# mikhaildubov/AST-text-analysis

Measured on AMD Instinct MI355X. Metric: corpus chars/sec (SA+annotation build + keyphrase score table), higher is better.
Workload: dtype u32 (symbols/indices) + f64 (scores); 1 GPU; 1 synthetic 64 MiB random-ASCII word-stream doc(s) per GPU (text mode), 1000 keyphrases, normalized scores, easa-HIP; symbols_per_gpu=61142967, strings_per_gpu=2982949, parallelism=doc-shard x1, all_gather_bytes_per_rank=0

## Files before the change

### ast-text-analysis_amd/csrc/build.h

```cpp
#pragma once
#include "dc3.h"
#include "score.h"
#include "tables.h"
#include "upload.h"
#include <chrono>

static bool kgram_reserve(east_hip_index *h, u64 bins, u32 n_docs);

static void annotate(east_hip_index *h, Ctx &ctx)
{
    const Pyramid &pyr = h->pyr;
    const u32 n = pyr.len[0];
    Arena &ar = *ctx.arena;
    const size_t mark = ar.mark();
    const u32 n_tiles = ceil_div_u32(n, ANN_TILE);
    u32 *wide_list = ar.alloc<u32>((size_t)n_tiles * ANN_TILE);
    u32 *wide_count = ar.alloc<u32>(n_tiles);
    const bool has_lvl1 = pyr.levels > 1;
    LAUNCH(ctx, ann_stream_kernel, n_tiles, pyr.ptr[0], (const u32 *)h->doc_off, (const u32 *)h->n_strings,
           h->build_docs, n, h->ann, has_lvl1 ? (u32 *)pyr.ptr[1] : (u32 *)nullptr, has_lvl1 ? pyr.len[1] : 0u,
           has_lvl1 ? pyr_padded(pyr.len[1]) : 0u, wide_list, wide_count, h->lcp);
    int l = 2;
    for (; l < pyr.levels && pyr.len[l] > PYR_TOP; l++)
        LAUNCH(ctx, pyramid_level_kernel, ceil_div_u32(pyr_padded(pyr.len[l]), BLOCK), pyr.ptr[l - 1], pyr.len[l],
               pyr_padded(pyr.len[l]), (u32 *)pyr.ptr[l]);
    if (l < pyr.levels) LAUNCH(ctx, pyramid_top_kernel, 1, pyr, l);
    LAUNCH(ctx, ann_wide_kernel, ceil_div_u32(n_tiles, BLOCK / ANN_WIDE_SLOTS), pyr, n, n_tiles, (const u32 *)wide_list,
           (const u32 *)wide_count, h->ann);
    ar.release(mark);
}

__global__ __launch_bounds__(BLOCK) void byte_hist_kernel(const uint8_t *__restrict__ s8, u32 n, u32 *__restrict__ counts)
{
    __shared__ u32 bins[4][256];
    for (int c = 0; c < 4; c++) bins[c][threadIdx.x] = 0;
    __syncthreads();
    u32 *mine = bins[threadIdx.x & 3u];
    for (u64 i = ((u64)blockIdx.x * BLOCK + threadIdx.x) * 16u; i < n; i += (u64)gridDim.x * BLOCK * 16u) {
        const uint4 x = *reinterpret_cast<const uint4 *>(s8 + i);
        const u32 wds[4] = {x.x, x.y, x.z, x.w};
#pragma unroll
        for (int q = 0; q < 16; q++)
            if (i + q < n) atomicAdd(&mine[(wds[q >> 2] >> ((q & 3) * 8)) & 0xFFu], 1u);
    }
    __syncthreads();
    const u32 t = bins[0][threadIdx.x] + bins[1][threadIdx.x] + bins[2][threadIdx.x] + bins[3][threadIdx.x];
    if (t) atomicAdd(&counts[threadIdx.x], t);
}

static void prepare_ht_code(east_hip_index *h, Ctx &ctx, u32 n, u32 sigma_t, u32 m_total)
{
    ctx.ht_max_len = 0;
    if (ctx.dry || !h->use_s8 || !ctx.knobs.window_sort || ctx.knobs.ht_mode == 0) return;
    if (ctx.spec) {
        if (!h->ht_valid || h->ht_sigma != sigma_t) {
            if (ctx.knobs.ht_mode == 1 && sigma_t + 1 >= 8 && n >= 64) throw SpecAbort();
            return;
        }
    } else {
        h->ht_valid = false;
        if (sigma_t + 1 < 8 || (ctx.knobs.ht_mode != 1 && (bit_width_u32(sigma_t + 1) < 6 || n < 65536)) || n < 64) return;
// ... 528 lines not shown
```

### ast-text-analysis_amd/csrc/debug_api.h

```cpp
#pragma once

struct DebugScope {
    hipStream_t stream = nullptr;
    Arena arena;
    Stats stats;
    Ctx ctx;
    DebugScope(int device, size_t bytes)
    {
        int c = 0;
        if (hipGetDeviceCount(&c) != hipSuccess || c <= 0)
            east_throw(EAST_HIP_ERR_NO_DEVICE, "no HIP device available (this library has no CPU fallback)");
        if (device < 0 || device >= c) east_throw(EAST_HIP_ERR_NO_DEVICE, "device ordinal out of range");
        use_device_ordinal(device);
        HIP_CHECK(hipStreamCreateWithFlags(&stream, hipStreamNonBlocking));
        void *p = nullptr;
        HIP_CHECK(hipMalloc(&p, bytes));
        arena.base = (char *)p;
        arena.cap = bytes;
        ctx.stream = stream;
        ctx.arena = &arena;
        ctx.stats = &stats;
    }
    ~DebugScope()
    {
// ... 35 lines not shown
    Arena &ar = sc.arena;
    u32 *d_sym = ar.alloc<u32>(n), *d_map = ar.alloc<u32>(TEXT_SYMBOLS);
    HIP_CHECK(hipMemcpyAsync(d_sym, symbols, (size_t)n * 4, hipMemcpyHostToDevice, sc.stream));
    HIP_CHECK(hipMemcpyAsync(d_map, code_map, TEXT_SYMBOLS * 4, hipMemcpyHostToDevice, sc.stream));
    for (int v = 0; v < 2; v++) {
        uint8_t *s8 = ar.alloc<uint8_t>((size_t)n + 64);
        u32 *present = ar.alloc<u32>(PRESENT_WORDS + 1), *hist = ar.alloc<u32>(hist_words), *group_sum = ar.alloc<u32>(sum_words);
        u32 *total = ar.alloc<u32>(total_words);
        HIP_CHECK(hipMemsetAsync(s8, v ? 0xA5 : 0x5A, (size_t)n + 64, sc.stream));
        HIP_CHECK(hipMemsetAsync(present, 0, (PRESENT_WORDS + 1) * 4, sc.stream));
        HIP_CHECK(hipMemsetAsync(hist, 0xEE, hist_words * 4, sc.stream));
        HIP_CHECK(hipMemsetAsync(group_sum, 0xEE, sum_words * 4, sc.stream));
        HIP_CHECK(hipMemsetAsync(total, 0, total_words * 4, sc.stream));
        const TextWindowGen<K> gen{s8, n, w, b, spare, term_first, DocKey()};
        if (v == 0) {
            LAUNCH_NAMED(sc.ctx, "presence_remap_hist_kernel", (presence_remap_hist_kernel<K, TextWindowGen<K>>), n_groups,
                         (const u32 *)d_sym, n, (const u32 *)d_map, present, s8, gen, shift, mask, n_tiles, hist, group_sum, total);
        } else {
            LAUNCH(sc.ctx, presence_kernel, std::min<u32>(ceil_div_u32(n, BLOCK), 2048), (const u32 *)d_sym, n, 1, present);
            LAUNCH(sc.ctx, remap_bytes_kernel, ceil_div_u32((u64)n + 16, BLOCK * 16), (const u32 *)d_sym, (const u32 *)d_map, n, 1, s8);
            hipLaunchKernelGGL((radix_hist_kernel<K, TextWindowGen<K>, false>), dim3(n_groups), dim3(RS_HIST_THREADS), 0, sc.stream, gen, n,
                               shift, mask, n_tiles, hist, group_sum, total, RsSeg());
            HIP_CHECK(hipGetLastError());
        }
        HIP_CHECK(hipMemcpyAsync(s8_out + (size_t)v * ((size_t)n + 16), s8, (size_t)n + 16, hipMemcpyDeviceToHost, sc.stream));
        HIP_CHECK(hipMemcpyAsync(present_out + (size_t)v * PRESENT_WORDS, present, PRESENT_WORDS * 4, hipMemcpyDeviceToHost, sc.stream));
        HIP_CHECK(hipMemcpyAsync(hist_out + v * hist_words, hist, hist_words * 4, hipMemcpyDeviceToHost, sc.stream));
        HIP_CHECK(hipMemcpyAsync(group_sum_out + v * sum_words, group_sum, sum_words * 4, hipMemcpyDeviceToHost, sc.stream));
        HIP_CHECK(hipMemcpyAsync(digit_total_out + v * total_words, total, total_words * 4, hipMemcpyDeviceToHost, sc.stream));
    }
    HIP_CHECK(hipStreamSynchronize(sc.stream));
}

extern "C" {

int east_hip_debug_set_rank_bucket_bytes(int64_t bytes)
{
    if (bytes < 0) return EAST_HIP_ERR_INVALID;
    knobs_update([&](Knobs &k) { k.rank_bucket_bytes = (size_t)bytes; k.plan_epoch++; });
    return EAST_HIP_OK;
}

int east_hip_debug_set_window_sort(int enabled)
{
    knobs_update([&](Knobs &k) {
    k.window_sort = enabled != 0;
    k.force_lean = enabled == 2;
    k.force_wide_keys = enabled == 3 || enabled == 5;
    k.fused_finish = enabled != 4 && enabled != 5 && enabled != 9 && getenv("EAST_HIP_NO_FUSED_FINISH") == nullptr;
    k.force_fused = enabled == 6 || getenv("EAST_HIP_FORCE_FUSED") != nullptr;
    k.ht_mode = enabled == 7 || enabled == 9 ? 1 : enabled == 8 ? 0 : env_int("EAST_HIP_HT", -1);
    k.plan_epoch++;
    });
    return EAST_HIP_OK;
}

int east_hip_debug_set_segmented_sort(int mode)
{
    knobs_update([&](Knobs &k) { k.seg_mode = mode < 0 ? env_int("EAST_HIP_SEG", -1) : (mode != 0); k.plan_epoch++; });
    return EAST_HIP_OK;
}

int east_hip_debug_alphabetic_code(const uint64_t *weights, int32_t n, uint32_t *code, int32_t *len)
{
    if (!weights || !code || !len || n < 1) return EAST_HIP_ERR_INVALID;
    std::vector<u64> w(weights, weights + n);
// ... 65 lines not shown

int east_hip_debug_set_text_stream(int64_t chunk_bytes)
{
    knobs_update([&](Knobs &k) { k.tp_stream = chunk_bytes; });
    return EAST_HIP_OK;
}

int east_hip_debug_set_score_path(int mode)
{
    knobs_update([&](Knobs &k) {
        k.kg_pairs = mode == 1 || mode == 2 || mode == 4 || mode == 5;
        k.kg_pairs_forced = mode == 4;
        k.score_fused = mode == 1 || mode == 3 || mode == 4 || mode == 5;
        k.score_endgame = mode == 5 ? 0 : 1;
    });
    return EAST_HIP_OK;
}

int east_hip_debug_set_speculation(int enabled)
{
    knobs_update([&](Knobs &k) { k.speculate = enabled != 0; k.first_hist = enabled != 2 && getenv("EAST_HIP_NO_FIRST_HIST") == nullptr; });
    return EAST_HIP_OK;
}

int east_hip_debug_first_pass_hist(int device, const uint32_t *symbols, int64_t n, const uint32_t *code_map, int key_bytes,
                                   int w, int b, int spare, uint32_t term_first, int shift, uint32_t mask, uint8_t *s8,
                                   uint32_t *present, uint32_t *hist, uint32_t *group_sum, uint32_t *digit_total)
{
    return guarded([&] {
        if (key_bytes == 8) debug_first_pass_hist<u64>(device, symbols, n, code_map, w, b, spare, term_first, shift, mask, s8, present, hist, group_sum, digit_total);
        else if (key_bytes == 4) debug_first_pass_hist<u32>(device, symbols, n, code_map, w, b, spare, term_first, shift, mask, s8, present, hist, group_sum, digit_total);
        else east_throw(EAST_HIP_ERR_INVALID, "key_bytes must be 4 or 8");
    });
}

int east_hip_debug_radix_sort_u64(int device, uint64_t *keys, uint32_t *vals, int64_t n, int bits)
{
    return guarded([&] { debug_sort<u64>(device, keys, vals, n, bits); });
}

int east_hip_debug_radix_sort_u32(int device, uint32_t *keys, uint32_t *vals, int64_t n, int bits)
{
    return guarded([&] { debug_sort<u32>(device, keys, vals, n, bits); });
}

int east_hip_debug_exclusive_scan(int device, const uint32_t *in, uint32_t *out, int64_t n)
{
    return guarded([&] {
        if (n < 0 || n >= (i64)0x7FFFFFF0 || !in || !out) east_throw(EAST_HIP_ERR_INVALID, "bad scan arguments");
        if (n == 0) return;
        DebugScope sc(device, (size_t)n * 8 + (size_t)ceil_div_u32(n, SCAN_TILE) * 16 + (8u << 20));
        u32 *d_in = sc.arena.alloc<u32>(n), *d_out = sc.arena.alloc<u32>(n);
        HIP_CHECK(hipMemcpyAsync(d_in, in, (size_t)n * 4, hipMemcpyHostToDevice, sc.stream));
        device_scan<ArrIn, false>(sc.ctx, ArrIn{d_in}, (u32)n, d_out);
        HIP_CHECK(hipMemcpyAsync(out, d_out, (size_t)n * 4, hipMemcpyDeviceToHost, sc.stream));
        HIP_CHECK(hipStreamSynchronize(sc.stream));
    });
}

int east_hip_debug_suffix_array(int device, const uint32_t *symbols, int64_t n, uint32_t sigma, int32_t *sa_out,
                                int32_t *levels_out)
{
    return guarded([&] {
        if (n < 1 || n >= (i64)0x7FFFFFF0 || !symbols || !sa_out || sigma < 1)
            east_throw(EAST_HIP_ERR_INVALID, "bad suffix array arguments");
        for (i64 i = 0; i < n; i++)
// ... 24 lines not shown
```

### ast-text-analysis_amd/csrc/tables.h

```cpp
#pragma once
#include "common.h"

#define PYR_SHIFT 4
#define PYR_FAN 16u
#define PYR_MAX_LEVELS 9
#define NONE_U32 0xFFFFFFFFu

struct Pyramid {
    const u32 *ptr[PYR_MAX_LEVELS];
    u32 len[PYR_MAX_LEVELS];
    int levels;
};

static inline u32 pyr_padded(u32 len) { return (len + PYR_FAN - 1u) & ~(PYR_FAN - 1u); }
__device__ __forceinline__ u32 pyr_padded_dev(u32 len) { return (len + PYR_FAN - 1u) & ~(PYR_FAN - 1u); }

__device__ __forceinline__ u32 doc_of(const u32 *__restrict__ doc_off, u32 n_docs, u32 x)
{
    u32 lo = 0, hi = n_docs;
    while (hi - lo > 1) {
        const u32 mid = (lo + hi) >> 1;
        if (doc_off[mid] <= x) lo = mid; else hi = mid;
    }
    return lo;
// ... 429 lines not shown
            rlvl--;
        }
    }
    pse = lq;
    nsv = rq;
}

__device__ __forceinline__ u32 pyr_leftmost_argmin(const Pyramid &P, u32 a, u32 b)
{
    const u32 lo = a + 1;
    u32 best = NONE_U32;
    {
        u32 l = lo, h = b;
        int lvl = 0;
        while (l < h) {
            const u32 *M = P.ptr[lvl];
            while (l < h && (l & (PYR_FAN - 1u))) { const u32 x = M[l]; best = x < best ? x : best; l++; }
            while (l < h && (h & (PYR_FAN - 1u))) { h--; const u32 x = M[h]; best = x < best ? x : best; }
            if (l >= h) break;
            if (lvl + 1 >= P.levels) {
                for (u32 q = l; q < h; q++) { const u32 x = M[q]; best = x < best ? x : best; }
                break;
            }
            l >>= PYR_SHIFT; h >>= PYR_SHIFT; lvl++;
        }
    }
    if (P.ptr[0][lo] == best) return lo;
    return pyr_find_right<false>(P, lo, best);
}

#ifndef ANN_NEAR
#define ANN_NEAR 8
#endif
#define ANN_IPT 4
#define ANN_TILE (BLOCK * ANN_IPT)
#ifndef ANN_HALO
#define ANN_HALO 64
#endif
#ifndef ANN_LOCAL
#define ANN_LOCAL 64
#endif

__global__ __launch_bounds__(BLOCK) void ann_stream_kernel(const u32 *__restrict__ lcp, const u32 *__restrict__ doc_off,
                                                           const u32 *__restrict__ n_strings, u32 n_docs, u32 n,
                                                           u32 *__restrict__ ann, u32 *__restrict__ lvl1, u32 len1,
                                                           u32 len1_padded, u32 *__restrict__ wide_list,
                                                           u32 *__restrict__ wide_count,
                                                           u32 *__restrict__ lcp_pad)
{
    __shared__ __attribute__((aligned(16))) u32 tile[ANN_TILE + 2 * ANN_HALO];
    __shared__ u32 work[ANN_TILE];
    __shared__ u32 work_count, far_count;
    if (threadIdx.x == 0) { work_count = 0; far_count = 0; }
    if (lcp_pad && blockIdx.x == gridDim.x - 1 && threadIdx.x < PYR_FAN && n + threadIdx.x < ((n + PYR_FAN - 1u) & ~(PYR_FAN - 1u)))
        lcp_pad[n + threadIdx.x] = NONE_U32;
    const u32 tile_base = blockIdx.x * ANN_TILE;
    const u32 k0 = tile_base + threadIdx.x * ANN_IPT;
    {
        uint4 x = {0u, 0u, 0u, 0u};
        if (k0 < ((n + PYR_FAN - 1u) & ~(PYR_FAN - 1u))) x = *reinterpret_cast<const uint4 *>(lcp + k0);
        if (k0 + 0 >= n) x.x = 0u;
        if (k0 + 1 >= n) x.y = 0u;
        if (k0 + 2 >= n) x.z = 0u;
        if (k0 + 3 >= n) x.w = 0u;
        const bool has_halo = threadIdx.x < 2 * ANN_HALO / 4;
        const bool left = threadIdx.x < ANN_HALO / 4;
        const u32 q = left ? threadIdx.x : threadIdx.x - ANN_HALO / 4;
        const i64 g = left ? (i64)tile_base - ANN_HALO + 4 * q : (i64)tile_base + ANN_TILE + 4 * q;
        uint4 h = {0u, 0u, 0u, 0u};
        if (has_halo && g >= 0 && g < (i64)((n + PYR_FAN - 1u) & ~(PYR_FAN - 1u))) h = *reinterpret_cast<const uint4 *>(lcp + g);
        *reinterpret_cast<uint4 *>(&tile[ANN_HALO + threadIdx.x * ANN_IPT]) = x;
        if (has_halo) {
            if (g + 0 >= (i64)n) h.x = 0u;
            if (g + 1 >= (i64)n) h.y = 0u;
            if (g + 2 >= (i64)n) h.z = 0u;
            if (g + 3 >= (i64)n) h.w = 0u;
            *reinterpret_cast<uint4 *>(&tile[left ? 4 * q : ANN_HALO + ANN_TILE + 4 * q]) = h;
        }
    }
    __syncthreads();
    if (threadIdx.x < ANN_TILE / PYR_FAN) {
        const u32 e = tile_base / PYR_FAN + threadIdx.x;
        if (e < len1_padded) {
            u32 m = NONE_U32;
            if (e < len1) {
                const uint4 *g = reinterpret_cast<const uint4 *>(&tile[ANN_HALO + threadIdx.x * PYR_FAN]);
#pragma unroll
                for (int q = 0; q < 4; q++) {
                    const uint4 y = g[q];
                    const u32 r = e * PYR_FAN + 4u * q;
                    if (r + 0 < n) m = min(m, y.x);
                    if (r + 1 < n) m = min(m, y.y);
                    if (r + 2 < n) m = min(m, y.z);
                    if (r + 3 < n) m = min(m, y.w);
                }
            }
            lvl1[e] = m;
        }
    }
    if (k0 < n) {
        u32 c[ANN_IPT + 2 * ANN_NEAR];
#pragma unroll
        for (int q = 0; q < (ANN_IPT + 2 * ANN_NEAR) / 4; q++) {
            const uint4 x = *reinterpret_cast<const uint4 *>(&tile[ANN_HALO + threadIdx.x * ANN_IPT - ANN_NEAR + 4 * q]);
            c[4 * q] = x.x; c[4 * q + 1] = x.y; c[4 * q + 2] = x.z; c[4 * q + 3] = x.w;
        }
        u32 out[ANN_IPT];
        bool direct[ANN_IPT];
#pragma unroll
        for (int e = 0; e < ANN_IPT; e++) {
            const u32 k = k0 + e;
            const int i = ANN_NEAR + e;
            const u32 v = c[i];
            out[e] = 0;
            direct[e] = true;
            if (k >= n) continue;
            if (v == 0) {
                const u32 d = n_docs > 1 ? doc_of(doc_off, n_docs, k) : 0u;
                out[e] = doc_off[d] == k ? (doc_off[d + 1] - k) - n_strings[d] : 0u;
                continue;
            }
            u32 back = 0, x = 0;
#pragma unroll
            for (int t = ANN_NEAR; t >= 1; t--)
                if (c[i - t] <= v) { back = (u32)t; x = c[i - t]; }
            if (back == 0) { direct[e] = false; continue; }
            if (x < v) {
                u32 fwd = 0;
#pragma unroll
                for (int t = ANN_NEAR; t >= 1; t--)
                    if (c[i + t] < v) fwd = (u32)t;
                if (fwd == 0) direct[e] = false;
                else out[e] = fwd + back;
            }
        }
        if (direct[0] && direct[1] && direct[2] && direct[3] && k0 + ANN_IPT <= n) {
            *reinterpret_cast<uint4 *>(ann + k0) = uint4{out[0], out[1], out[2], out[3]};
        } else {
#pragma unroll
            for (int e = 0; e < ANN_IPT; e++) {
                if (k0 + e >= n) break;
                if (direct[e]) ann[k0 + e] = out[e];
                else work[atomicAdd(&work_count, 1u)] = threadIdx.x * ANN_IPT + e;
            }
        }
    }
    __syncthreads();
    const u32 count = work_count;
    const u32 sub = threadIdx.x & 7u;
    for (u32 wi = threadIdx.x >> 3; wi < count; wi += BLOCK / 8) {
        const u32 local = work[wi], at = ANN_HALO + local;
        const u32 v = tile[at];
        constexpr u32 NONE_D = ANN_LOCAL + 1;
        u32 d = NONE_D;
#pragma unroll
        for (u32 t = 0; t < (ANN_LOCAL + 7) / 8; t++) {
            const u32 dist = 1u + sub + 8u * t;
            if (dist <= ANN_LOCAL && d == NONE_D && tile[at - dist] <= v) d = dist;
        }
        d = min(d, (u32)__shfl_xor((int)d, 1, 8));
        d = min(d, (u32)__shfl_xor((int)d, 2, 8));
        d = min(d, (u32)__shfl_xor((int)d, 4, 8));
        bool far = d == NONE_D;
        u32 a = 0;
        if (!far && tile[at - d] < v) {
            u32 e = NONE_D;
#pragma unroll
            for (u32 t = 0; t < (ANN_LOCAL + 7) / 8; t++) {
                const u32 dist = 1u + sub + 8u * t;
                if (dist <= ANN_LOCAL && e == NONE_D && tile[at + dist] < v) e = dist;
            }
            e = min(e, (u32)__shfl_xor((int)e, 1, 8));
            e = min(e, (u32)__shfl_xor((int)e, 2, 8));
            e = min(e, (u32)__shfl_xor((int)e, 4, 8));
            if (e == NONE_D) far = true;
            else a = d + e;
        }
        if (sub == 0) {
            if (far) wide_list[tile_base + atomicAdd(&far_count, 1u)] = tile_base + local;
            else ann[tile_base + local] = a;
        }
    }
    __syncthreads();
    if (threadIdx.x == 0) wide_count[blockIdx.x] = far_count;
}

#define ANN_WIDE_SLOTS 16
__global__ __launch_bounds__(BLOCK) void ann_wide_kernel(Pyramid P, u32 n, u32 n_tiles, const u32 *__restrict__ wide_list,
                                                         const u32 *__restrict__ wide_count, u32 *__restrict__ ann)
{
    const u32 *lcp = P.ptr[0];
    const u32 tile = blockIdx.x * (BLOCK / ANN_WIDE_SLOTS) + threadIdx.x / ANN_WIDE_SLOTS;
    if (tile >= n_tiles) return;
    const u32 count = wide_count[tile];
    for (u32 i = threadIdx.x % ANN_WIDE_SLOTS; i < count; i += ANN_WIDE_SLOTS) {
        const u32 k = wide_list[tile * ANN_TILE + i];
        const u32 v = lcp[k];
        u32 pse, nsv;
        pyr_find_both(P, k, v, pse, nsv);
        u32 a = 0;
        if (pse != NONE_U32 && lcp[pse] < v) a = (nsv == NONE_U32 ? n : nsv) - pse;
        ann[k] = a;
    }
}

#define CH_NEAR 8
#ifndef CH_HALO
#define CH_HALO 64
#endif
#ifndef CH_LOCAL
#define CH_LOCAL 64
#endif
#define CH_IPT 4
#define CH_TILE (BLOCK * CH_IPT)

__device__ __forceinline__ void child_of_rank(const Pyramid &P, u32 k, u32 seg, u32 seg_end, u32 &u, u32 &dn, u32 &nx)
{
    const u32 *lcp = P.ptr[0];
    const u32 v = lcp[k];
    u32 pse = NONE_U32, nse = NONE_U32;
    if (k > seg) {
        pse = pyr_find_left<false>(P, k, v);
        if (pse != NONE_U32 && pse < seg) pse = NONE_U32;
    }
    nse = pyr_find_right<false>(P, k, v);
    if (nse != NONE_U32 && nse >= seg_end) nse = NONE_U32;
    nx = (nse != NONE_U32 && lcp[nse] == v) ? nse - seg : 0u;
    u = dn = 0;
    if (pse != NONE_U32 && k - pse > 1) u = pyr_leftmost_argmin(P, pse, k) - seg;
    if (nse != NONE_U32 && nse - k > 1) dn = pyr_leftmost_argmin(P, k, nse) - seg;
}

__global__ __launch_bounds__(BLOCK) void child_stream_kernel(Pyramid P, const u32 *__restrict__ doc_off, u32 n_docs, u32 n,
                                                             u32 *__restrict__ up, u32 *__restrict__ down,
                                                             u32 *__restrict__ next, u32 *__restrict__ wide_list,
                                                             u32 *__restrict__ wide_count)
{
// ... 228 lines not shown
```

### ast-text-analysis_amd/east/hip_backend.py

```python
import atexit
import ctypes
import os

import numpy as np

from east import exceptions

_HERE = os.path.dirname(os.path.abspath(__file__))
LIB_PATH = os.environ.get("EAST_HIP_LIBRARY", os.path.join(_HERE, "_lib", "libeast_hip.so"))

_c_i64p = ctypes.POINTER(ctypes.c_int64)
_c_i32p = ctypes.POINTER(ctypes.c_int32)
_c_u32p = ctypes.POINTER(ctypes.c_uint32)
_c_u64p = ctypes.POINTER(ctypes.c_uint64)
_c_dblp = ctypes.POINTER(ctypes.c_double)

SIGNATURES = {
    "east_hip_version": (ctypes.c_char_p, []),
    "east_hip_last_error": (ctypes.c_char_p, []),
    "east_hip_device_count": (ctypes.c_int, []),
    "east_hip_create": (ctypes.c_int, [ctypes.c_int, ctypes.c_int64, ctypes.POINTER(ctypes.c_void_p)]),
    "east_hip_reset": (ctypes.c_int, [ctypes.c_void_p]),
    "east_hip_destroy": (None, [ctypes.c_void_p]),
    "east_hip_build": (ctypes.c_int, [ctypes.c_void_p, _c_u32p, ctypes.c_int64, _c_i64p, _c_i32p, ctypes.c_int32]),
# ... 11 lines not shown
    "east_hip_last_prep_ms": (ctypes.c_double, [ctypes.c_void_p]),
    "east_hip_get_tables": (ctypes.c_int, [ctypes.c_void_p, ctypes.c_int32] + [_c_i32p] * 6),
    "east_hip_score_table": (ctypes.c_int, [ctypes.c_void_p, _c_u32p, _c_i64p, ctypes.c_int32, ctypes.c_int,
                                            _c_dblp, _c_dblp]),
    "east_hip_score_table_grouped": (ctypes.c_int, [ctypes.c_void_p, _c_u32p, _c_i64p, ctypes.c_int32, _c_i64p,
                                                    ctypes.c_int32, ctypes.c_int, _c_dblp]),
    "east_hip_get_lcp_intervals": (ctypes.c_int, [ctypes.c_void_p, ctypes.c_int32, _c_i32p]),
    "east_hip_set_keyphrases": (ctypes.c_int, [ctypes.c_void_p, _c_u32p, _c_i64p, ctypes.c_int32]),
    "east_hip_score_resident": (ctypes.c_int, [ctypes.c_void_p, ctypes.c_int, ctypes.c_void_p]),
    "east_hip_score_probes": (ctypes.c_int, [ctypes.c_void_p, ctypes.c_int, _c_i64p]),
    "east_hip_score_resident_async": (ctypes.c_int, [ctypes.c_void_p, ctypes.c_int]),
    "east_hip_synchronize": (ctypes.c_int, [ctypes.c_void_p]),
    "east_hip_stream": (ctypes.c_void_p, [ctypes.c_void_p]),
    "east_hip_build_info": (ctypes.c_int, [ctypes.c_void_p, _c_i64p, ctypes.c_int32]),
    "east_hip_last_build_ms": (ctypes.c_double, [ctypes.c_void_p]),
    "east_hip_last_score_ms": (ctypes.c_double, [ctypes.c_void_p]),
    "east_hip_debug_radix_sort_u64": (ctypes.c_int, [ctypes.c_int, _c_u64p, _c_u32p, ctypes.c_int64, ctypes.c_int]),
    "east_hip_debug_radix_sort_u32": (ctypes.c_int, [ctypes.c_int, _c_u32p, _c_u32p, ctypes.c_int64, ctypes.c_int]),
    "east_hip_debug_exclusive_scan": (ctypes.c_int, [ctypes.c_int, _c_u32p, _c_u32p, ctypes.c_int64]),
    "east_hip_debug_suffix_array": (ctypes.c_int, [ctypes.c_int, _c_u32p, ctypes.c_int64, ctypes.c_uint32, _c_i32p,
                                                   _c_i32p]),
    "east_hip_plan_arena_bytes": (ctypes.c_int64, [ctypes.c_int64, ctypes.c_int32]),
    "east_hip_plan_arena_bytes_lean": (ctypes.c_int64, [ctypes.c_int64, ctypes.c_int32]),
    "east_hip_debug_set_rank_bucket_bytes": (ctypes.c_int, [ctypes.c_int64]),
    "east_hip_debug_set_window_sort": (ctypes.c_int, [ctypes.c_int]),
    "east_hip_debug_set_lds_rounds": (ctypes.c_int, [ctypes.c_int]),
    "east_hip_debug_set_persist": (ctypes.c_int, [ctypes.c_int, ctypes.c_int]),
    "east_hip_debug_set_segmented_sort": (ctypes.c_int, [ctypes.c_int]),
    "east_hip_debug_set_speculation": (ctypes.c_int, [ctypes.c_int]),
    "east_hip_debug_first_pass_hist": (ctypes.c_int, [ctypes.c_int, _c_u32p, ctypes.c_int64, _c_u32p, ctypes.c_int,
                                                      ctypes.c_int, ctypes.c_int, ctypes.c_int, ctypes.c_uint32, ctypes.c_int,
                                                      ctypes.c_uint32, ctypes.POINTER(ctypes.c_uint8), _c_u32p, _c_u32p,
                                                      _c_u32p, _c_u32p]),
    "east_hip_debug_set_score_scratch": (ctypes.c_int, [ctypes.c_int64]),
    "east_hip_debug_set_score_path": (ctypes.c_int, [ctypes.c_int]),
    "east_hip_debug_set_score_grid": (ctypes.c_int, [ctypes.c_int64]),
    "east_hip_debug_set_text_stream": (ctypes.c_int, [ctypes.c_int64]),
    "east_hip_debug_set_text_ring": (ctypes.c_int, [ctypes.c_int, ctypes.c_int64]),
    "east_hip_debug_alphabetic_code": (ctypes.c_int, [ctypes.POINTER(ctypes.c_uint64), ctypes.c_int32,
                                                      ctypes.POINTER(ctypes.c_uint32), ctypes.POINTER(ctypes.c_int32)]),
    "east_hip_debug_narrow_symbols": (ctypes.c_int, [_c_u32p, ctypes.c_int64, ctypes.POINTER(ctypes.c_uint16), ctypes.c_int]),
    "east_hip_debug_narrow_symbols8": (ctypes.c_int, [_c_u32p, ctypes.c_int64, ctypes.POINTER(ctypes.c_uint8), ctypes.c_int]),
    "east_hip_group_create": (ctypes.c_int, [_c_i32p, ctypes.c_int32, ctypes.POINTER(ctypes.c_void_p)]),
    "east_hip_group_destroy": (None, [ctypes.c_void_p]),
    "east_hip_group_build": (ctypes.c_int, [ctypes.c_void_p, _c_u32p, ctypes.c_int64, _c_i64p, _c_i32p, ctypes.c_int32,
                                            ctypes.c_int32]),
    "east_hip_group_build_texts_v": (ctypes.c_int, [ctypes.c_void_p, ctypes.POINTER(ctypes.c_char_p), _c_i64p, ctypes.c_int32,
                                                    ctypes.POINTER(ctypes.c_uint8), _c_u32p, _c_u32p, _c_u32p, _c_u32p,
                                                    _c_u32p, ctypes.c_int32]),
    "east_hip_group_shards": (ctypes.c_int, [ctypes.c_void_p, _c_i32p]),
    "east_hip_group_handle": (ctypes.c_void_p, [ctypes.c_void_p, ctypes.c_int32]),
    "east_hip_score_table_multi": (ctypes.c_int, [ctypes.c_void_p, _c_u32p, _c_i64p, ctypes.c_int32, ctypes.c_int, _c_dblp]),
    "east_hip_group_info": (ctypes.c_int, [ctypes.c_void_p, _c_dblp, ctypes.c_int32]),
    "east_hip_debug_shard_documents": (ctypes.c_int, [_c_i64p, ctypes.c_int32, ctypes.c_int32, _c_i32p]),
    "east_hip_format_table_xml": (ctypes.c_int64, [_c_dblp, ctypes.c_int32, ctypes.c_int32, _c_i32p, _c_i32p,
                                                   ctypes.POINTER(ctypes.c_char_p), ctypes.POINTER(ctypes.c_char_p),
                                                   ctypes.c_char_p, ctypes.c_int64]),
    "east_hip_format_table_csv": (ctypes.c_int64, [_c_dblp, ctypes.c_int32, ctypes.c_int32, _c_i32p, _c_i32p,
                                                   ctypes.POINTER(ctypes.c_char_p), ctypes.POINTER(ctypes.c_char_p),
                                                   ctypes.c_char_p, ctypes.c_int64]),
    "east_hip_profile_enable": (ctypes.c_int, [ctypes.c_void_p, ctypes.c_int]),
    "east_hip_profile_only": (ctypes.c_int, [ctypes.c_void_p, ctypes.c_char_p]),
    "east_hip_profile_report": (ctypes.c_int64, [ctypes.c_void_p, ctypes.c_char_p, ctypes.c_int64]),
    "east_hip_cosine_build_texts": (ctypes.c_int, [ctypes.c_void_p, ctypes.c_char_p, ctypes.c_int64, _c_i64p, ctypes.c_int32,
                                                   ctypes.POINTER(ctypes.c_uint8), _c_u32p, _c_u32p, _c_u32p, _c_u32p,
                                                   _c_u32p, ctypes.c_int32, _c_u32p, _c_i64p, ctypes.c_int32]),
# ... 773 lines not shown
```

### include/east_hip.h

```cpp
#ifndef EAST_HIP_H
#define EAST_HIP_H

#include <stdint.h>

#ifdef __cplusplus
extern "C" {
#endif

#define EAST_HIP_OK                 0
#define EAST_HIP_ERR_NO_DEVICE     -1
#define EAST_HIP_ERR_INVALID       -2
#define EAST_HIP_ERR_OOM           -3
#define EAST_HIP_ERR_HIP           -4
#define EAST_HIP_ERR_DOMAIN        -5
#define EAST_HIP_ERR_NOT_BUILT     -6
#define EAST_HIP_ERR_INTERNAL      -7

#define EAST_HIP_TERMINATOR_START 0x0A00u
#define EAST_HIP_TERMINATOR_TAG   0x80000000u
#define EAST_HIP_SYMBOLS_REFERENCE 0
#define EAST_HIP_SYMBOLS_TAGGED    1

typedef struct east_hip_index *east_hip_handle_t;

// ... 117 lines not shown
int east_hip_debug_shard_documents(const int64_t *sizes, int32_t n_docs, int32_t n_shards, int32_t *first_doc);

int64_t east_hip_format_table_xml(const double *table, int32_t K, int32_t D, const int32_t *kp_order, const int32_t *text_order,
                                  const char *const *kp_names, const char *const *text_names, char *out, int64_t cap);
int64_t east_hip_format_table_csv(const double *table, int32_t K, int32_t D, const int32_t *kp_order, const int32_t *text_order,
                                  const char *const *kp_quoted, const char *const *text_quoted, char *out, int64_t cap);

int east_hip_synchronize(east_hip_handle_t h);
void *east_hip_stream(east_hip_handle_t h);

int east_hip_build_info(east_hip_handle_t h, int64_t *out, int32_t cap);

double east_hip_last_build_ms(east_hip_handle_t h);
double east_hip_last_score_ms(east_hip_handle_t h);

int east_hip_profile_enable(east_hip_handle_t h, int on);
int east_hip_profile_only(east_hip_handle_t h, const char *kernel);
int64_t east_hip_profile_report(east_hip_handle_t h, char *buf, int64_t cap);

int east_hip_debug_radix_sort_u64(int device, uint64_t *keys, uint32_t *vals, int64_t n, int bits);
int east_hip_debug_radix_sort_u32(int device, uint32_t *keys, uint32_t *vals, int64_t n, int bits);
int east_hip_debug_exclusive_scan(int device, const uint32_t *in, uint32_t *out, int64_t n);
int east_hip_debug_suffix_array(int device, const uint32_t *symbols, int64_t n, uint32_t sigma,
                                int32_t *sa_out, int32_t *levels_out);
int east_hip_debug_set_rank_bucket_bytes(int64_t bytes);
int east_hip_debug_set_window_sort(int enabled);
int east_hip_debug_set_segmented_sort(int mode);
int east_hip_debug_set_persist(int force_large, int max_workgroups);
int east_hip_debug_set_lds_rounds(int enabled);
int east_hip_debug_set_speculation(int enabled);
int east_hip_debug_first_pass_hist(int device, const uint32_t *symbols, int64_t n, const uint32_t *code_map, int key_bytes,
                                   int w, int b, int spare, uint32_t term_first, int shift, uint32_t mask, uint8_t *s8,
                                   uint32_t *present, uint32_t *hist, uint32_t *group_sum, uint32_t *digit_total);
int east_hip_debug_set_score_scratch(int64_t bytes);
int east_hip_debug_set_score_grid(int64_t workgroups);
int east_hip_debug_set_text_stream(int64_t chunk_bytes);
int east_hip_debug_set_text_ring(int mode, int64_t slot_bytes);
int east_hip_debug_set_term_hash_bits(int bits);
int east_hip_debug_set_synonyms_chunk(int entries);
int east_hip_debug_set_top_tile(int members);
int east_hip_debug_alphabetic_code(const uint64_t *weights, int32_t n, uint32_t *code, int32_t *len);
int east_hip_debug_narrow_symbols(const uint32_t *symbols, int64_t n, uint16_t *out, int vector);
int east_hip_debug_narrow_symbols8(const uint32_t *symbols, int64_t n, uint8_t *out, int vector);
int east_hip_debug_set_score_path(int mode);
int64_t east_hip_plan_arena_bytes(int64_t n_total, int32_t n_docs);
int64_t east_hip_plan_arena_bytes_lean(int64_t n_total, int32_t n_docs);

#ifdef __cplusplus
}
#endif
#endif
```

Baseline: 40.74 billion chars/s.

## Rework LCP annotation with group-min window search and balanced wide pass

The annotation stream kernel now handles larger tiles (8 items per thread, wider halo). It builds per-16-element group minima plus prefix and suffix minima in LDS, so nearest smaller-value searches cover the whole window with ballots instead of a fixed 64-element local scan, and fewer items fall back to the global pyramid path. The level-1 minima reuse these group minima. The wide fallback kernel now load-balances: it scans counts over runs of 64 tiles and splits the combined work across 8 slices per run, rather than giving each tile a fixed 16 lanes. A debug annotate entry point is added for testing, at the cost of more LDS per block and more complex kernels.

Measured after the change: 42.30 billion chars/s, median of 6. 1.04x the previous value.

```diff
diff --git a/ast-text-analysis_amd/csrc/build.h b/ast-text-analysis_amd/csrc/build.h
--- a/ast-text-analysis_amd/csrc/build.h
+++ b/ast-text-analysis_amd/csrc/build.h
@@ -7,7 +7,7 @@
 
 static bool kgram_reserve(east_hip_index *h, u64 bins, u32 n_docs);
 
-static void annotate(east_hip_index *h, Ctx &ctx)
+static void annotate(east_hip_index *h, Ctx &ctx, u32 *listed_total = nullptr)
 {
     const Pyramid &pyr = h->pyr;
     const u32 n = pyr.len[0];
@@ -25,8 +25,8 @@
         LAUNCH(ctx, pyramid_level_kernel, ceil_div_u32(pyr_padded(pyr.len[l]), BLOCK), pyr.ptr[l - 1], pyr.len[l],
                pyr_padded(pyr.len[l]), (u32 *)pyr.ptr[l]);
     if (l < pyr.levels) LAUNCH(ctx, pyramid_top_kernel, 1, pyr, l);
-    LAUNCH(ctx, ann_wide_kernel, ceil_div_u32(n_tiles, BLOCK / ANN_WIDE_SLOTS), pyr, n, n_tiles, (const u32 *)wide_list,
-           (const u32 *)wide_count, h->ann);
+    LAUNCH(ctx, ann_wide_kernel, ceil_div_u32(n_tiles, ANN_WIDE_RUN) * ANN_WIDE_SLICES, pyr, n, n_tiles, (const u32 *)wide_list,
+           (const u32 *)wide_count, h->ann, listed_total);
     ar.release(mark);
 }
 
diff --git a/ast-text-analysis_amd/csrc/debug_api.h b/ast-text-analysis_amd/csrc/debug_api.h
--- a/ast-text-analysis_amd/csrc/debug_api.h
+++ b/ast-text-analysis_amd/csrc/debug_api.h
@@ -91,6 +91,53 @@
     HIP_CHECK(hipStreamSynchronize(sc.stream));
 }
 
+static void debug_annotate(int device, const u32 *lcp, i64 n64, const i64 *doc_off, int32_t n_docs, const int32_t *n_strings,
+                           u32 *ann_out, u32 *geometry_out, u32 *listed_out)
+{
+    if (!lcp || !doc_off || !n_strings || !ann_out || !geometry_out || !listed_out || n64 < 1 || n64 >= (i64)0x7FFFFFF0 ||
+        n_docs < 1 || doc_off[0] != 0 || doc_off[n_docs] != n64)
+        east_throw(EAST_HIP_ERR_INVALID, "bad annotation arguments");
+    for (int32_t d = 0; d < n_docs; d++)
+        if (doc_off[d + 1] <= doc_off[d]) east_throw(EAST_HIP_ERR_INVALID, "document offsets must increase");
+    const u32 n = (u32)n64;
+    std::vector<u32> off32((size_t)n_docs + 1), m32(n_docs);
+    for (int32_t d = 0; d <= n_docs; d++) off32[d] = (u32)doc_off[d];
+    for (int32_t d = 0; d < n_docs; d++) m32[d] = (u32)n_strings[d];
+    DebugScope sc(device, ((size_t)pyr_padded(n) * 2 + (size_t)n / 8 + (size_t)ceil_div_u32(n, ANN_TILE) * (ANN_TILE + 1) + 2 * (size_t)n_docs) * 4 +
+                              (1u << 20));
+    Arena &ar = sc.arena;
+    east_hip_index h;
+    h.lcp = ar.alloc<u32>(pyr_padded(n));
+    h.ann = ar.alloc<u32>(n);
+    h.doc_off = ar.alloc<u32>((size_t)n_docs + 1);
+    h.n_strings = ar.alloc<u32>(n_docs);
+    h.build_docs = (u32)n_docs;
+    u32 *listed = ar.alloc<u32>(1);
+    Pyramid &pyr = h.pyr;
+    pyr.levels = 1;
+    pyr.ptr[0] = h.lcp;
+    pyr.len[0] = n;
+    while (pyr.len[pyr.levels - 1] > PYR_FAN) {
+        const u32 len = ceil_div_u32(pyr.len[pyr.levels - 1], PYR_FAN);
+        pyr.ptr[pyr.levels] = ar.alloc<u32>(pyr_padded(len));
+        pyr.len[pyr.levels] = len;
+        pyr.levels++;
+    }
+    HIP_CHECK(hipMemsetAsync(h.lcp, 0x5A, (size_t)pyr_padded(n) * 4, sc.stream));
+    HIP_CHECK(hipMemsetAsync(h.ann, 0xEE, (size_t)n * 4, sc.stream));
+    HIP_CHECK(hipMemsetAsync(listed, 0, 4, sc.stream));
+    HIP_CHECK(hipMemcpyAsync(h.lcp, lcp, (size_t)n * 4, hipMemcpyHostToDevice, sc.stream));
+    HIP_CHECK(hipMemcpyAsync(h.doc_off, off32.data(), off32.size() * 4, hipMemcpyHostToDevice, sc.stream));
+    HIP_CHECK(hipMemcpyAsync(h.n_strings, m32.data(), m32.size() * 4, hipMemcpyHostToDevice, sc.stream));
+    annotate(&h, sc.ctx, listed);
+    HIP_CHECK(hipMemcpyAsync(ann_out, h.ann, (size_t)n * 4, hipMemcpyDeviceToHost, sc.stream));
+    HIP_CHECK(hipMemcpyAsync(listed_out, listed, 4, hipMemcpyDeviceToHost, sc.stream));
+    HIP_CHECK(hipStreamSynchronize(sc.stream));
+    geometry_out[0] = ANN_TILE;
+    geometry_out[1] = ANN_HALO;
+    geometry_out[2] = ANN_NEAR;
+}
+
 extern "C" {
 
 int east_hip_debug_set_rank_bucket_bytes(int64_t bytes)
@@ -222,6 +269,12 @@
         else if (key_bytes == 4) debug_first_pass_hist<u32>(device, symbols, n, code_map, w, b, spare, term_first, shift, mask, s8, present, hist, group_sum, digit_total);
         else east_throw(EAST_HIP_ERR_INVALID, "key_bytes must be 4 or 8");
     });
+}
+
+int east_hip_debug_annotate(int device, const uint32_t *lcp, int64_t n, const int64_t *doc_off, int32_t n_docs,
+                            const int32_t *n_strings, uint32_t *ann_out, uint32_t *geometry_out, uint32_t *listed_out)
+{
+    return guarded([&] { debug_annotate(device, lcp, n, doc_off, n_docs, n_strings, ann_out, geometry_out, listed_out); });
 }
 
 int east_hip_debug_radix_sort_u64(int device, uint64_t *keys, uint32_t *vals, int64_t n, int bits)
diff --git a/ast-text-analysis_amd/csrc/tables.h b/ast-text-analysis_amd/csrc/tables.h
--- a/ast-text-analysis_amd/csrc/tables.h
+++ b/ast-text-analysis_amd/csrc/tables.h
@@ -485,14 +485,48 @@
 #ifndef ANN_NEAR
 #define ANN_NEAR 8
 #endif
-#define ANN_IPT 4
+#ifndef ANN_IPT
+#define ANN_IPT 8
+#endif
+#define ANN_QUADS (ANN_IPT / 4)
 #define ANN_TILE (BLOCK * ANN_IPT)
 #ifndef ANN_HALO
-#define ANN_HALO 64
+#define ANN_HALO 128
 #endif
-#ifndef ANN_LOCAL
-#define ANN_LOCAL 64
-#endif
+#define ANN_WINDOW (ANN_TILE + 2 * ANN_HALO)
+#define ANN_GROUPS (ANN_WINDOW / PYR_FAN)
+#define ANN_GROUPS_PER_LANE ((ANN_GROUPS + 63) / 64)
+static_assert(ANN_IPT == 4 || ANN_IPT == 8, "a thread holds one or two quads");
+static_assert(ANN_HALO % PYR_FAN == 0 && ANN_HALO >= ANN_NEAR + 4 && 2 * ANN_HALO / 4 <= BLOCK, "the halo: whole groups, one quad per thread");
+static_assert(ANN_TILE <= 65536, "the work list holds 16-bit tile offsets");
+
+__device__ __forceinline__ u32 ann_ballot8(bool pred, u32 sh) { return (u32)(__ballot(pred) >> sh) & 0xFFu; }
+
+template <bool LEFT>
+__device__ __forceinline__ u32 ann_window_search(const u32 *tile, const u32 *gmin, const u32 *gedge, bool want, u32 at,
+                                                 u32 v, u32 own, u32 sub, u32 sh)
+{
+    const u32 g = at >> PYR_SHIFT, o = at & (PYR_FAN - 1u);
+    u32 m = LEFT ? own & ((1u << o) - 1u) : own & ~((2u << o) - 1u);
+    u32 grp = g;
+    bool walk = want && !m && (LEFT ? gedge[g] <= v : gedge[g] < v);
+    for (u32 t = 0; t < (ANN_GROUPS + 7) / 8 && __ballot(walk) != 0; t++) {
+        const u32 c = LEFT ? g - 1u - sub - 8u * t : g + 1u + sub + 8u * t;
+        const u32 x = gmin[c < ANN_GROUPS ? c : 0u];
+        const u32 h = ann_ballot8(walk && c < ANN_GROUPS && (LEFT ? x <= v : x < v), sh);
+        if (walk && h) {
+            const u32 s = (u32)__ffs((int)h) - 1u;
+            grp = LEFT ? g - 1u - 8u * t - s : g + 1u + 8u * t + s;
+            walk = false;
+        }
+    }
+    const bool fetch = want && grp != g;
+    const u32 y0 = tile[(grp << PYR_SHIFT) + sub], y1 = tile[(grp << PYR_SHIFT) + 8u + sub];
+    const u32 far = ann_ballot8(fetch && (LEFT ? y0 <= v : y0 < v), sh) | ann_ballot8(fetch && (LEFT ? y1 <= v : y1 < v), sh) << 8;
+    if (fetch) m = far;
+    if (!want || !m) return NONE_U32;
+    return (grp << PYR_SHIFT) + (LEFT ? 31u - (u32)__clz((int)m) : (u32)__ffs((int)m) - 1u);
+}
 
 __global__ __launch_bounds__(BLOCK) void ann_stream_kernel(const u32 *__restrict__ lcp, const u32 *__restrict__ doc_off,
                                                            const u32 *__restrict__ n_strings, u32 n_docs, u32 n,
@@ -501,67 +535,110 @@
                                                            u32 *__restrict__ wide_count,
                                                            u32 *__restrict__ lcp_pad)
 {
-    __shared__ __attribute__((aligned(16))) u32 tile[ANN_TILE + 2 * ANN_HALO];
-    __shared__ u32 work[ANN_TILE];
+    __shared__ __attribute__((aligned(16))) u32 tile[ANN_WINDOW];
+    __shared__ u32 gmin[ANN_GROUPS], gbefore[ANN_GROUPS], gbehind[ANN_GROUPS];
+    __shared__ uint16_t work[ANN_TILE];
     __shared__ u32 work_count, far_count;
     if (threadIdx.x == 0) { work_count = 0; far_count = 0; }
-    if (lcp_pad && blockIdx.x == gridDim.x - 1 && threadIdx.x < PYR_FAN && n + threadIdx.x < ((n + PYR_FAN - 1u) & ~(PYR_FAN - 1u)))
+    const u32 n_padded = pyr_padded_dev(n);
+    if (lcp_pad && blockIdx.x == gridDim.x - 1 && threadIdx.x < PYR_FAN && n + threadIdx.x < n_padded)
         lcp_pad[n + threadIdx.x] = NONE_U32;
     const u32 tile_base = blockIdx.x * ANN_TILE;
-    const u32 k0 = tile_base + threadIdx.x * ANN_IPT;
     {
-        uint4 x = {0u, 0u, 0u, 0u};
-        if (k0 < ((n + PYR_FAN - 1u) & ~(PYR_FAN - 1u))) x = *reinterpret_cast<const uint4 *>(lcp + k0);
-        if (k0 + 0 >= n) x.x = 0u;
-        if (k0 + 1 >= n) x.y = 0u;
-        if (k0 + 2 >= n) x.z = 0u;
-        if (k0 + 3 >= n) x.w = 0u;
+        uint4 x[ANN_QUADS];
+#pragma unroll
+        for (int j = 0; j < ANN_QUADS; j++) {
+            const u32 k0 = tile_base + (u32)j * 4u * BLOCK + threadIdx.x * 4u;
+            x[j] = uint4{0u, 0u, 0u, 0u};
+            if (k0 < n_padded) x[j] = *reinterpret_cast<const uint4 *>(lcp + k0);
+        }
         const bool has_halo = threadIdx.x < 2 * ANN_HALO / 4;
         const bool left = threadIdx.x < ANN_HALO / 4;
         const u32 q = left ? threadIdx.x : threadIdx.x - ANN_HALO / 4;
         const i64 g = left ? (i64)tile_base - ANN_HALO + 4 * q : (i64)tile_base + ANN_TILE + 4 * q;
         uint4 h = {0u, 0u, 0u, 0u};
-        if (has_halo && g >= 0 && g < (i64)((n + PYR_FAN - 1u) & ~(PYR_FAN - 1u))) h = *reinterpret_cast<const uint4 *>(lcp + g);
-        *reinterpret_cast<uint4 *>(&tile[ANN_HALO + threadIdx.x * ANN_IPT]) = x;
+        if (has_halo && g >= 0 && g < (i64)n_padded) h = *reinterpret_cast<const uint4 *>(lcp + g);
+#pragma unroll
+        for (int j = 0; j < ANN_QUADS; j++) {
+            const u32 local0 = (u32)j * 4u * BLOCK + threadIdx.x * 4u, k0 = tile_base + local0;
+            if (k0 + 0 >= n) x[j].x = 0u;
+            if (k0 + 1 >= n) x[j].y = 0u;
+            if (k0 + 2 >= n) x[j].z = 0u;
+            if (k0 + 3 >= n) x[j].w = 0u;
+            *reinterpret_cast<uint4 *>(&tile[ANN_HALO + local0]) = x[j];
+            u32 m = min(min(x[j].x, x[j].y), min(x[j].z, x[j].w));
+            m = min(m, (u32)__shfl_xor((int)m, 1));
+            m = min(m, (u32)__shfl_xor((int)m, 2));
+            if ((threadIdx.x & 3u) == 0) gmin[(ANN_HALO + local0) >> PYR_SHIFT] = m;
+        }
+        if (g + 0 >= (i64)n) h.x = 0u;
+        if (g + 1 >= (i64)n) h.y = 0u;
+        if (g + 2 >= (i64)n) h.z = 0u;
+        if (g + 3 >= (i64)n) h.w = 0u;
+        const u32 at = left ? 4 * q : ANN_HALO + ANN_TILE + 4 * q;
+        u32 m = min(min(h.x, h.y), min(h.z, h.w));
+        m = min(m, (u32)__shfl_xor((int)m, 1));
+        m = min(m, (u32)__shfl_xor((int)m, 2));
         if (has_halo) {
-            if (g + 0 >= (i64)n) h.x = 0u;
-            if (g + 1 >= (i64)n) h.y = 0u;
-            if (g + 2 >= (i64)n) h.z = 0u;
-            if (g + 3 >= (i64)n) h.w = 0u;
-            *reinterpret_cast<uint4 *>(&tile[left ? 4 * q : ANN_HALO + ANN_TILE + 4 * q]) = h;
+            *reinterpret_cast<uint4 *>(&tile[at]) = h;
+            if ((threadIdx.x & 3u) == 0) gmin[at >> PYR_SHIFT] = m;
         }
     }
     __syncthreads();
-    if (threadIdx.x < ANN_TILE / PYR_FAN) {
-        const u32 e = tile_base / PYR_FAN + threadIdx.x;
+    if (wave_id() < 2) {
+        const bool fwd = wave_id() == 0;
+        const u32 lane = lane_id();
+        u32 mine[ANN_GROUPS_PER_LANE], all = NONE_U32;
+#pragma unroll
+        for (u32 i = 0; i < ANN_GROUPS_PER_LANE; i++) {
+            const u32 gi = lane * ANN_GROUPS_PER_LANE + i;
+            mine[i] = gi < ANN_GROUPS ? gmin[gi] : NONE_U32;
+            all = min(all, mine[i]);
+        }
+        u32 inc = all;
+#pragma unroll
+        for (u32 d = 1; d < 64; d <<= 1) {
+            const u32 other = fwd ? (u32)__shfl_up((int)inc, d) : (u32)__shfl_down((int)inc, d);
+            if (fwd ? lane >= d : lane + d < 64u) inc = min(inc, other);
+        }
+        u32 run = fwd ? (u32)__shfl_up((int)inc, 1) : (u32)__shfl_down((int)inc, 1);
+        if (fwd ? lane == 0 : lane == 63u) run = NONE_U32;
+#pragma unroll
+        for (u32 i = 0; i < ANN_GROUPS_PER_LANE; i++) {
+            const u32 ii = fwd ? i : ANN_GROUPS_PER_LANE - 1u - i;
+            const u32 gi = lane * ANN_GROUPS_PER_LANE + ii;
+            if (gi < ANN_GROUPS) (fwd ? gbefore : gbehind)[gi] = run;
+            run = min(run, mine[ii]);
+        }
+    }
+    if (threadIdx.x >= BLOCK - ANN_TILE / PYR_FAN) {
+        const u32 i = threadIdx.x - (BLOCK - ANN_TILE / PYR_FAN);
+        const u32 e = tile_base / PYR_FAN + i;
         if (e < len1_padded) {
             u32 m = NONE_U32;
             if (e < len1) {
-                const uint4 *g = reinterpret_cast<const uint4 *>(&tile[ANN_HALO + threadIdx.x * PYR_FAN]);
-#pragma unroll
-                for (int q = 0; q < 4; q++) {
-                    const uint4 y = g[q];
-                    const u32 r = e * PYR_FAN + 4u * q;
-                    if (r + 0 < n) m = min(m, y.x);
-                    if (r + 1 < n) m = min(m, y.y);
-                    if (r + 2 < n) m = min(m, y.z);
-                    if (r + 3 < n) m = min(m, y.w);
+                if ((e + 1u) * PYR_FAN <= n) m = gmin[ANN_HALO / PYR_FAN + i];
+                else {
+                    for (u32 r = e * PYR_FAN; r < n; r++) m = min(m, tile[ANN_HALO + (r - tile_base)]);
                 }
             }
             lvl1[e] = m;
         }
     }
-    if (k0 < n) {
-        u32 c[ANN_IPT + 2 * ANN_NEAR];
-#pragma unroll
-        for (int q = 0; q < (ANN_IPT + 2 * ANN_NEAR) / 4; q++) {
-            const uint4 x = *reinterpret_cast<const uint4 *>(&tile[ANN_HALO + threadIdx.x * ANN_IPT - ANN_NEAR + 4 * q]);
+#pragma unroll
+    for (int j = 0; j < ANN_QUADS; j++) {
+        const u32 local0 = (u32)j * 4u * BLOCK + threadIdx.x * 4u, k0 = tile_base + local0;
+        if (k0 >= n) continue;
+        u32 c[4 + 2 * ANN_NEAR];
+#pragma unroll
+        for (int q = 0; q < (4 + 2 * ANN_NEAR) / 4; q++) {
+            const uint4 x = *reinterpret_cast<const uint4 *>(&tile[ANN_HALO + local0 - ANN_NEAR + 4 * q]);
             c[4 * q] = x.x; c[4 * q + 1] = x.y; c[4 * q + 2] = x.z; c[4 * q + 3] = x.w;
         }
-        u32 out[ANN_IPT];
-        bool direct[ANN_IPT];
-#pragma unroll
-        for (int e = 0; e < ANN_IPT; e++) {
+        u32 out[4];
+        bool direct[4];
+#pragma unroll
+        for (int e = 0; e < 4; e++) {
             const u32 k = k0 + e;
             const int i = ANN_NEAR + e;
             const u32 v = c[i];
@@ -587,67 +664,71 @@
                 else out[e] = fwd + back;
             }
         }
-        if (direct[0] && direct[1] && direct[2] && direct[3] && k0 + ANN_IPT <= n) {
+        if (direct[0] && direct[1] && direct[2] && direct[3] && k0 + 4 <= n) {
             *reinterpret_cast<uint4 *>(ann + k0) = uint4{out[0], out[1], out[2], out[3]};
         } else {
 #pragma unroll
-            for (int e = 0; e < ANN_IPT; e++) {
+            for (int e = 0; e < 4; e++) {
                 if (k0 + e >= n) break;
                 if (direct[e]) ann[k0 + e] = out[e];
-                else work[atomicAdd(&work_count, 1u)] = threadIdx.x * ANN_IPT + e;
+                else work[atomicAdd(&work_count, 1u)] = (uint16_t)(local0 + e);
             }
         }
     }
     __syncthreads();
     const u32 count = work_count;
-    const u32 sub = threadIdx.x & 7u;
-    for (u32 wi = threadIdx.x >> 3; wi < count; wi += BLOCK / 8) {
-        const u32 local = work[wi], at = ANN_HALO + local;
+    const u32 sub = threadIdx.x & 7u, sh = lane_id() & 56u;
+    for (u32 first_wi = 0; first_wi < count; first_wi += BLOCK / 8) {
+        const u32 wi = first_wi + (threadIdx.x >> 3);
+        const bool on = wi < count;
+        const u32 local = on ? work[wi] : 0u, at = ANN_HALO + local;
         const u32 v = tile[at];
-        constexpr u32 NONE_D = ANN_LOCAL + 1;
-        u32 d = NONE_D;
-#pragma unroll
-        for (u32 t = 0; t < (ANN_LOCAL + 7) / 8; t++) {
-            const u32 dist = 1u + sub + 8u * t;
-            if (dist <= ANN_LOCAL && d == NONE_D && tile[at - dist] <= v) d = dist;
-        }
-        d = min(d, (u32)__shfl_xor((int)d, 1, 8));
-        d = min(d, (u32)__shfl_xor((int)d, 2, 8));
-        d = min(d, (u32)__shfl_xor((int)d, 4, 8));
-        bool far = d == NONE_D;
-        u32 a = 0;
-        if (!far && tile[at - d] < v) {
-            u32 e = NONE_D;
-#pragma unroll
-            for (u32 t = 0; t < (ANN_LOCAL + 7) / 8; t++) {
-                const u32 dist = 1u + sub + 8u * t;
-                if (dist <= ANN_LOCAL && e == NONE_D && tile[at + dist] < v) e = dist;
-            }
-            e = min(e, (u32)__shfl_xor((int)e, 1, 8));
-            e = min(e, (u32)__shfl_xor((int)e, 2, 8));
-            e = min(e, (u32)__shfl_xor((int)e, 4, 8));
-            if (e == NONE_D) far = true;
-            else a = d + e;
-        }
-        if (sub == 0) {
-            if (far) wide_list[tile_base + atomicAdd(&far_count, 1u)] = tile_base + local;
-            else ann[tile_base + local] = a;
+        const u32 g0 = at & ~(PYR_FAN - 1u);
+        const u32 y0 = tile[g0 + sub], y1 = tile[g0 + 8u + sub];
+        const u32 le = ann_ballot8(y0 <= v, sh) | ann_ballot8(y1 <= v, sh) << 8;
+        const u32 lt = ann_ballot8(y0 < v, sh) | ann_ballot8(y1 < v, sh) << 8;
+        const u32 p = ann_window_search<true>(tile, gmin, gbefore, on, at, v, le, sub, sh);
+        const bool first = on && p != NONE_U32 && tile[p] < v;
+        const u32 q = ann_window_search<false>(tile, gmin, gbehind, first, at, v, lt, sub, sh);
+        if (on && sub == 0) {
+            if (p == NONE_U32 || (first && q == NONE_U32)) wide_list[tile_base + atomicAdd(&far_count, 1u)] = tile_base + local;
+            else ann[tile_base + local] = first ? q - p : 0u;
         }
     }
     __syncthreads();
     if (threadIdx.x == 0) wide_count[blockIdx.x] = far_count;
 }
 
-#define ANN_WIDE_SLOTS 16
+#define ANN_WIDE_RUN 64
+#define ANN_WIDE_SLICES 8
 __global__ __launch_bounds__(BLOCK) void ann_wide_kernel(Pyramid P, u32 n, u32 n_tiles, const u32 *__restrict__ wide_list,
-                                                         const u32 *__restrict__ wide_count, u32 *__restrict__ ann)
-{
+                                                         const u32 *__restrict__ wide_count, u32 *__restrict__ ann,
+                                                         u32 *__restrict__ listed_total)
+{
+    __shared__ u32 off[ANN_WIDE_RUN + 1];
     const u32 *lcp = P.ptr[0];
-    const u32 tile = blockIdx.x * (BLOCK / ANN_WIDE_SLOTS) + threadIdx.x / ANN_WIDE_SLOTS;
-    if (tile >= n_tiles) return;
-    const u32 count = wide_count[tile];
-    for (u32 i = threadIdx.x % ANN_WIDE_SLOTS; i < count; i += ANN_WIDE_SLOTS) {
-        const u32 k = wide_list[tile * ANN_TILE + i];
+    const u32 tile0 = blockIdx.x / ANN_WIDE_SLICES * ANN_WIDE_RUN, slice = blockIdx.x % ANN_WIDE_SLICES;
+    if (threadIdx.x < ANN_WIDE_RUN) {
+        const u32 t = tile0 + threadIdx.x;
+        u32 inc = t < n_tiles ? wide_count[t] : 0u;
+#pragma unroll
+        for (u32 d = 1; d < ANN_WIDE_RUN; d <<= 1) {
+            const u32 other = (u32)__shfl_up((int)inc, d);
+            if (threadIdx.x >= d) inc += other;
+        }
+        off[threadIdx.x + 1] = inc;
+        if (threadIdx.x == 0) off[0] = 0;
+    }
+    __syncthreads();
+    const u32 total = off[ANN_WIDE_RUN];
+    if (listed_total && slice == 0 && threadIdx.x == 0 && total) atomicAdd(listed_total, total);
+    for (u32 j = slice * BLOCK + threadIdx.x; j < total; j += ANN_WIDE_SLICES * BLOCK) {
+        u32 lo = 0, hi = ANN_WIDE_RUN;
+        while (hi - lo > 1) {
+            const u32 mid = (lo + hi) >> 1;
+            if (off[mid] <= j) lo = mid; else hi = mid;
+        }
+        const u32 k = wide_list[(size_t)(tile0 + lo) * ANN_TILE + (j - off[lo])];
         const u32 v = lcp[k];
         u32 pse, nsv;
         pyr_find_both(P, k, v, pse, nsv);
@@ -656,6 +737,7 @@
         ann[k] = a;
     }
 }
+static_assert(ANN_WIDE_RUN == 64, "one wavefront scans a run's counts");
 
 #define CH_NEAR 8
 #ifndef CH_HALO
diff --git a/ast-text-analysis_amd/east/hip_backend.py b/ast-text-analysis_amd/east/hip_backend.py
--- a/ast-text-analysis_amd/east/hip_backend.py
+++ b/ast-text-analysis_amd/east/hip_backend.py
@@ -67,6 +67,8 @@
                                                       ctypes.c_int, ctypes.c_int, ctypes.c_int, ctypes.c_uint32, ctypes.c_int,
                                                       ctypes.c_uint32, ctypes.POINTER(ctypes.c_uint8), _c_u32p, _c_u32p,
                                                       _c_u32p, _c_u32p]),
+    "east_hip_debug_annotate": (ctypes.c_int, [ctypes.c_int, _c_u32p, ctypes.c_int64, _c_i64p, ctypes.c_int32, _c_i32p,
+                                               _c_u32p, _c_u32p, _c_u32p]),
     "east_hip_debug_set_score_scratch": (ctypes.c_int, [ctypes.c_int64]),
     "east_hip_debug_set_score_path": (ctypes.c_int, [ctypes.c_int]),
     "east_hip_debug_set_score_grid": (ctypes.c_int, [ctypes.c_int64]),
diff --git a/include/east_hip.h b/include/east_hip.h
--- a/include/east_hip.h
+++ b/include/east_hip.h
@@ -173,6 +173,8 @@
 int east_hip_debug_first_pass_hist(int device, const uint32_t *symbols, int64_t n, const uint32_t *code_map, int key_bytes,
                                    int w, int b, int spare, uint32_t term_first, int shift, uint32_t mask, uint8_t *s8,
                                    uint32_t *present, uint32_t *hist, uint32_t *group_sum, uint32_t *digit_total);
+int east_hip_debug_annotate(int device, const uint32_t *lcp, int64_t n, const int64_t *doc_off, int32_t n_docs,
+                            const int32_t *n_strings, uint32_t *ann_out, uint32_t *geometry_out, uint32_t *listed_out);
 int east_hip_debug_set_score_scratch(int64_t bytes);
 int east_hip_debug_set_score_grid(int64_t workgroups);
 int east_hip_debug_set_text_stream(int64_t chunk_bytes);
```
